# sahaRatul/sela

Hardware: AMD Instinct MI355X
Metric: Msamples/s encode+decode, 16-bit stereo 44.1kHz, 1/2/4/8 GPU; bit-exact vs CPU (higher is better)
Workload: dtype f64+int64

## Files before the change

### sela_amd/csrc/sela_synth.h

```cpp
#ifndef SELA_SYNTH_H_
#define SELA_SYNTH_H_

#include "sela_device.h"

namespace sela {

typedef const volatile __attribute__((address_space(3))) uint64_t* LdsTable;

__device__ __forceinline__ int32_t rice_value(uint32_t ones, uint32_t field, uint32_t k)
{
    const uint32_t rem = k ? (__brev(field) >> (32 - k)) : 0u;
    const uint32_t u = (ones << k) | rem;
    return (int32_t)((u >> 1) ^ (0u - (u & 1u)));
}

struct StreamWords {
    const uint32_t* words;
    uint32_t n_words;
};
__device__ __forceinline__ __amdgpu_buffer_rsrc_t stream_rsrc(const StreamWords& s)
{
    return __builtin_amdgcn_make_buffer_rsrc(
        reinterpret_cast<void*>(read_first_lane(reinterpret_cast<uint64_t>(s.words))), 0,
        4u * (uint32_t)__builtin_amdgcn_readfirstlane((int)s.n_words), 0x00020000);
}
__device__ __forceinline__ void window64(__amdgpu_buffer_rsrc_t rs, uint32_t p, uint32_t& x0, uint32_t& x1)
{
    const uint32_t b = 4 * (p >> 5), sh = p & 31;
    const uint32_t w0 = __builtin_amdgcn_raw_buffer_load_b32(rs, b, 0, 0), w1 = __builtin_amdgcn_raw_buffer_load_b32(rs, b + 4, 0, 0),
                   w2 = __builtin_amdgcn_raw_buffer_load_b32(rs, b + 8, 0, 0);
    x0 = __builtin_amdgcn_alignbit(w1, w0, sh);
    x1 = __builtin_amdgcn_alignbit(w2, w1, sh);
}

template <bool kFold, bool kShift>
__device__ __forceinline__ void synth_mac(uint32_t& zl, uint32_t& zh, uint64_t coef, int32_t s_i, int32_t& shifted)
{
    const int32_t al = (int32_t)(uint32_t)coef, ah = (int32_t)(uint32_t)(coef >> 32);
    const uint64_t z = ((uint64_t)zh << 32) | zl;
    const uint64_t lo = (uint64_t)((int64_t)z + (int64_t)al * (int64_t)s_i);
    if (kFold) {
        if (kShift)
            asm("v_mad_i32_i24 %0, %2, %3, %4\n\tv_ashrrev_i32 %1, 3, %0" : "=v"(zh), "=v"(shifted) : "v"(ah), "s"(s_i), "v"((uint32_t)(lo >> 32)));
        else
            asm("v_mad_i32_i24 %0, %1, %2, %3" : "=v"(zh) : "v"(ah), "s"(s_i), "v"((uint32_t)(lo >> 32)));
    } else {
        zh = (uint32_t)(lo >> 32) + (uint32_t)ah * (uint32_t)s_i;
        if (kShift) {
            shifted = (int32_t)zh >> 3;
            asm volatile("" : "+v"(shifted));
        }
    }
    zl = (uint32_t)lo;
}

constexpr int kAhead = 4;

template <int R, bool kFold, int G, bool kVecShift, int M>
__device__ __forceinline__ void synth_steps(uint32_t& cl, uint32_t& ch, uint32_t& ol, uint32_t& oh, uint32_t& kept,
    LdsTable tab_lane, int32_t r_block, uint32_t four, uint32_t zero, uint64_t (&pf_c)[kAhead], uint64_t (&pf_o)[kAhead], int32_t& shifted)
{
    const int32_t pred = kVecShift ? __builtin_amdgcn_readlane(shifted, M) : __builtin_amdgcn_readlane((int)ch, M) >> 3;
    int32_t m_i;
    if (kFold)
        m_i = pred;
    else
        m_i = (int32_t)((uint32_t)pred - (uint32_t)__builtin_amdgcn_readlane(r_block, M));
    synth_mac<kFold, kVecShift>(cl, ch, pf_c[M % kAhead], m_i, shifted);
    if (R == 2) {
        int32_t unused;
        synth_mac<kFold, false>(ol, oh, pf_o[M % kAhead], m_i, unused);
    }
    if constexpr (M + kAhead < 64) {
        pf_c[M % kAhead] = tab_lane[64 * R - (M + kAhead)];
        if (R == 2)
            pf_o[M % kAhead] = tab_lane[64 - (M + kAhead)];
    }
    if constexpr ((M + 1) % G == 0) {
        constexpr int first_lane = M + 1 - G;
        constexpr int row_mask = 1 << (first_lane / 16);
        constexpr int bank_mask = G == 16 ? 0xf : 1 << ((first_lane % 16) / 4);
        kept = (uint32_t)__builtin_amdgcn_update_dpp((int)kept, (int)ch, 0xE4 , row_mask, bank_mask, false);
        ch = (uint32_t)__builtin_amdgcn_update_dpp((int)ch, (int)four, 0xE4, row_mask, bank_mask, false);
        cl = (uint32_t)__builtin_amdgcn_update_dpp((int)cl, (int)zero, 0xE4, row_mask, bank_mask, false);
    }
    __builtin_amdgcn_sched_barrier(0);
    if constexpr (M < 63)
        synth_steps<R, kFold, G, kVecShift, M + 1>(cl, ch, ol, oh, kept, tab_lane, r_block, four, zero, pf_c, pf_o, shifted);
}

template <int R, bool kFold, int G, bool kVecShift>
__device__ __forceinline__ bool synth_block(int32_t r_block, int32_t& s, uint32_t& cl, uint32_t& ch, uint32_t& ol, uint32_t& oh,
    LdsTable tab_lane, uint32_t four, uint32_t zero)
{
    uint64_t pf_c[kAhead], pf_o[kAhead];
#pragma unroll
    for (int m = 0; m < kAhead; m++) {
        pf_c[m] = tab_lane[64 * R - m];
        pf_o[m] = R == 2 ? tab_lane[64 - m] : 0;
    }
    if (kFold)
        ch -= (uint32_t)r_block << 3;
    uint32_t kept = 0;
    int32_t shifted = 0;
    if (kVecShift) {
        shifted = (int32_t)ch >> 3;
        asm volatile("" : "+v"(shifted));
    }
    __builtin_amdgcn_sched_barrier(0);
    synth_steps<R, kFold, G, kVecShift, 0>(cl, ch, ol, oh, kept, tab_lane, r_block, four, zero, pf_c, pf_o, shifted);
    s = (int32_t)((kFold ? 0u : (uint32_t)r_block) - (uint32_t)((int32_t)kept >> 3));
    return !kFold || !__any((uint32_t)(s + (1 << 23) - 1) >= (1u << 24) - 1u);
}

template <bool kOut32>
struct SynthOut {
};
template <>
struct SynthOut<true> {
    int32_t* samples;
    uint32_t n;
};

template <int R, int G, bool kVecShift, bool kOut32 = false>
__device__ __attribute__((noinline)) void synthesize(
    const uint32_t* words, uint32_t n_words, uint32_t k, uint16_t* pos_smp, const int32_t* ws,
    const uint64_t* tab, bool fold, int lane, SynthOut<kOut32> out32 = SynthOut<kOut32>())
{
    static_assert(G == 4 || G == 16, "groups are DPP banks or rows");
    const StreamWords sw = { words, n_words };
    const __amdgpu_buffer_rsrc_t rs = stream_rsrc(sw);
    k = (uint32_t)__builtin_amdgcn_readfirstlane((int)k);
    const uint32_t kmask = k ? (0xFFFFFFFFu >> (32 - k)) : 0u;
    const bool jit = read_first_lane(reinterpret_cast<uint64_t>(ws)) == 0;
    uint32_t zl[2], zh[2];
#pragma unroll
    for (int h = 0; h < 2; h++) {
        zl[h] = 0;
        zh[h] = 4;
    }
    uint32_t four = 4, zero = 0;
    asm volatile("" : "+v"(four), "+v"(zero));
    const LdsTable tab_lane = (LdsTable)(tab + lane);
    uint32_t p = 0, w0 = 0, w1 = 0, w2 = 0;
    int32_t r_ws = 0;
    uint32_t n_samples = (uint32_t)kBlock;
    if constexpr (kOut32)
        n_samples = (uint32_t)__builtin_amdgcn_readfirstlane((int)out32.n);
    const int n_blocks = kOut32 ? (int)((n_samples + 63) / 64) : kBlock / 64;
    auto issue = [&](int blk) {
        if (jit) {
            p = pos_smp[64 * blk + lane];
            const uint32_t b = 4 * (p >> 5);
            w0 = __builtin_amdgcn_raw_buffer_load_b32(rs, b, 0, 0);
            w1 = __builtin_amdgcn_raw_buffer_load_b32(rs, b + 4, 0, 0);
            w2 = __builtin_amdgcn_raw_buffer_load_b32(rs, b + 8, 0, 0);
        } else if constexpr (kOut32) {
            r_ws = (uint32_t)(64 * blk + lane) < n_samples ? ws[64 * blk + lane] : 0;
        } else {
            w2 = (uint32_t)ws[64 * blk + lane];
        }
    };
    auto land = [&]() -> int32_t {
        if (!jit)
            return kOut32 ? r_ws : (int32_t)w2;
        uint32_t x0 = __builtin_amdgcn_alignbit(w1, w0, p & 31), x1 = __builtin_amdgcn_alignbit(w2, w1, p & 31), ones = 0;
        while (__any(x0 == 0xFFFFFFFFu)) {
            const bool more = x0 == 0xFFFFFFFFu;
            ones += more ? 32u : 0u;
            p += more ? 32u : 0u;
            window64(rs, p, x0, x1);
        }
        const uint32_t t = (uint32_t)__builtin_ctz(~x0);
        const uint32_t field = (uint32_t)(((((uint64_t)x1) << 32) | x0) >> (t + 1)) & kmask;
        return rice_value(ones + t, field, k);
    };
    auto run_block = [&](int blk, uint32_t& cl, uint32_t& ch, uint32_t& ol, uint32_t& oh) {
        const int32_t r_block = land();
        if (blk + 1 < n_blocks)
            issue(blk + 1);
        int32_t s;
        bool done = false;
        fold = fold && !__any((uint32_t)(r_block + (1 << 23) - 1) >= (1u << 24) - 1u);
        if (fold) {
            const uint32_t s0 = cl, s1 = ch, s2 = ol, s3 = oh;
            done = synth_block<R, true, G, kVecShift>(r_block, s, cl, ch, ol, oh, tab_lane, four, zero);
            if (!done) {
                cl = s0, ch = s1;
                if (R == 2)
                    ol = s2, oh = s3;
                fold = false;
            }
        }
        if (!done)
            synth_block<R, false, G, kVecShift>(r_block, s, cl, ch, ol, oh, tab_lane, four, zero);
        if constexpr (kOut32) {
            if ((uint32_t)(64 * blk + lane) < n_samples)
                out32.samples[64 * blk + lane] = s;
        } else
            reinterpret_cast<int16_t*>(pos_smp)[64 * blk + lane] = (int16_t)(uint16_t)(uint32_t)s;
    };
    if (n_blocks > 0)
        issue(0);
    if constexpr (kOut32) {
#pragma unroll 1
        for (int pair = 0; pair < n_blocks; pair += R) {
            run_block(pair, zl[0], zh[0], zl[R - 1], zh[R - 1]);
            if (R == 2 && pair + 1 < n_blocks)
                run_block(pair + 1, zl[1], zh[1], zl[0], zh[0]);
        }
    } else {
#pragma unroll 1
        for (int blk = 0; blk < n_blocks; blk++) {
            run_block(blk, zl[0], zh[0], zl[R - 1], zh[R - 1]);
            if (R == 2) {
                const uint32_t tl = zl[0], th = zh[0];
                zl[0] = zl[1], zh[0] = zh[1];
                zl[1] = tl, zh[1] = th;
            }
        }
    }
    wave_sync();
}

template <bool kVecShift, bool kOut32 = false>
__device__ __forceinline__ void synthesize_by_order(uint32_t order, const uint32_t* words, uint32_t n_words, uint32_t k, uint16_t* pos_smp,
    const int32_t* ws, const uint64_t* tab, bool fold, int lane, SynthOut<kOut32> out32 = SynthOut<kOut32>())
{
    if (order <= 48)
        synthesize<1, 16, kVecShift, kOut32>(words, n_words, k, pos_smp, ws, tab, fold, lane, out32);
    else if (order <= 60)
        synthesize<1, 4, kVecShift, kOut32>(words, n_words, k, pos_smp, ws, tab, fold, lane, out32);
    else
        synthesize<2, 16, kVecShift, kOut32>(words, n_words, k, pos_smp, ws, tab, fold, lane, out32);
}

__device__ inline bool build_synth_table(const int64_t* a, uint64_t* tab, int order, int lane)
{
    uint64_t c[2];
    bool fits = true;
#pragma unroll
    for (int h = 0; h < 2; h++) {
        const int d = lane + 64 * h;
        const uint64_t nv = (uint64_t)(d >= 1 && d <= order ? a[d] : 0);
        const int32_t al = (int32_t)(uint32_t)nv;
        const int32_t ah = (int32_t)(uint32_t)((nv - (uint64_t)(int64_t)al) >> 32);
        fits &= ah >= -(1 << 23) && ah < (1 << 23);
        c[h] = ((uint64_t)(uint32_t)ah << 32) | (uint32_t)al;
    }
    wave_sync();
    if (order <= 60) {
        tab[lane] = c[0];
        tab[lane + 64] = c[0];
    } else {
        tab[lane] = c[0];
        tab[lane + 64] = c[1];
        tab[lane + 128] = c[0];
    }
    wave_sync();
    return !__any(!fits);
}

}

#endif
```

Baseline: 18080.

## Recycle synth lanes via exec-masked moves, add 8-lane groups, streamline rice decode

In the non-out32 path, lane recycling now sets exec with s_bfm_b64 and uses a 64-bit v_mov to restore the accumulator pair, replacing three DPP updates. A G=8 group size is added for orders 49-56, so the lane-recycling granularity can match the order more closely. The rice decode in the jit path also drops the mask and branch on k. The trade-offs are reliance on inline asm that writes exec directly, and a k==0 shift edge case in the new rice code.

```diff
diff --git a/sela_amd/csrc/sela_synth.h b/sela_amd/csrc/sela_synth.h
--- a/sela_amd/csrc/sela_synth.h
+++ b/sela_amd/csrc/sela_synth.h
@@ -54,11 +54,16 @@
     zl = (uint32_t)lo;
 }
 
+struct Restart {
+    uint32_t four, zero;
+    uint64_t sum;
+};
+
 constexpr int kAhead = 4;
 
-template <int R, bool kFold, int G, bool kVecShift, int M>
+template <int R, bool kFold, int G, bool kVecShift, bool kDppRecycle, int M>
 __device__ __forceinline__ void synth_steps(uint32_t& cl, uint32_t& ch, uint32_t& ol, uint32_t& oh, uint32_t& kept,
-    LdsTable tab_lane, int32_t r_block, uint32_t four, uint32_t zero, uint64_t (&pf_c)[kAhead], uint64_t (&pf_o)[kAhead], int32_t& shifted)
+    LdsTable tab_lane, int32_t r_block, const Restart& restart, uint64_t (&pf_c)[kAhead], uint64_t (&pf_o)[kAhead], int32_t& shifted)
 {
     const int32_t pred = kVecShift ? __builtin_amdgcn_readlane(shifted, M) : __builtin_amdgcn_readlane((int)ch, M) >> 3;
     int32_t m_i;
@@ -78,20 +83,29 @@
     }
     if constexpr ((M + 1) % G == 0) {
         constexpr int first_lane = M + 1 - G;
-        constexpr int row_mask = 1 << (first_lane / 16);
-        constexpr int bank_mask = G == 16 ? 0xf : 1 << ((first_lane % 16) / 4);
-        kept = (uint32_t)__builtin_amdgcn_update_dpp((int)kept, (int)ch, 0xE4 , row_mask, bank_mask, false);
-        ch = (uint32_t)__builtin_amdgcn_update_dpp((int)ch, (int)four, 0xE4, row_mask, bank_mask, false);
-        cl = (uint32_t)__builtin_amdgcn_update_dpp((int)cl, (int)zero, 0xE4, row_mask, bank_mask, false);
+        if constexpr (kDppRecycle) {
+            constexpr int row_mask = 1 << (first_lane / 16);
+            constexpr int bank_mask = G == 16 ? 0xf : G == 8 ? 0x3 << ((first_lane % 16) / 8 * 2) : 1 << ((first_lane % 16) / 4);
+            kept = (uint32_t)__builtin_amdgcn_update_dpp((int)kept, (int)ch, 0xE4 , row_mask, bank_mask, false);
+            ch = (uint32_t)__builtin_amdgcn_update_dpp((int)ch, (int)restart.four, 0xE4, row_mask, bank_mask, false);
+            cl = (uint32_t)__builtin_amdgcn_update_dpp((int)cl, (int)restart.zero, 0xE4, row_mask, bank_mask, false);
+        } else {
+            uint64_t c = ((uint64_t)ch << 32) | cl;
+            asm volatile("s_bfm_b64 exec, %4, %5\n\tv_mov_b32 %1, %2\n\tv_mov_b64 %0, %3\n\ts_mov_b64 exec, -1"
+                         : "+v"(c), "+v"(kept)
+                         : "v"(ch), "s"(restart.sum), "n"(G), "n"(first_lane));
+            cl = (uint32_t)c;
+            ch = (uint32_t)(c >> 32);
+        }
     }
     __builtin_amdgcn_sched_barrier(0);
     if constexpr (M < 63)
-        synth_steps<R, kFold, G, kVecShift, M + 1>(cl, ch, ol, oh, kept, tab_lane, r_block, four, zero, pf_c, pf_o, shifted);
-}
-
-template <int R, bool kFold, int G, bool kVecShift>
+        synth_steps<R, kFold, G, kVecShift, kDppRecycle, M + 1>(cl, ch, ol, oh, kept, tab_lane, r_block, restart, pf_c, pf_o, shifted);
+}
+
+template <int R, bool kFold, int G, bool kVecShift, bool kDppRecycle>
 __device__ __forceinline__ bool synth_block(int32_t r_block, int32_t& s, uint32_t& cl, uint32_t& ch, uint32_t& ol, uint32_t& oh,
-    LdsTable tab_lane, uint32_t four, uint32_t zero)
+    LdsTable tab_lane, const Restart& restart)
 {
     uint64_t pf_c[kAhead], pf_o[kAhead];
 #pragma unroll
@@ -108,7 +122,7 @@
         asm volatile("" : "+v"(shifted));
     }
     __builtin_amdgcn_sched_barrier(0);
-    synth_steps<R, kFold, G, kVecShift, 0>(cl, ch, ol, oh, kept, tab_lane, r_block, four, zero, pf_c, pf_o, shifted);
+    synth_steps<R, kFold, G, kVecShift, kDppRecycle, 0>(cl, ch, ol, oh, kept, tab_lane, r_block, restart, pf_c, pf_o, shifted);
     s = (int32_t)((kFold ? 0u : (uint32_t)r_block) - (uint32_t)((int32_t)kept >> 3));
     return !kFold || !__any((uint32_t)(s + (1 << 23) - 1) >= (1u << 24) - 1u);
 }
@@ -127,7 +141,7 @@
     const uint32_t* words, uint32_t n_words, uint32_t k, uint16_t* pos_smp, const int32_t* ws,
     const uint64_t* tab, bool fold, int lane, SynthOut<kOut32> out32 = SynthOut<kOut32>())
 {
-    static_assert(G == 4 || G == 16, "groups are DPP banks or rows");
+    static_assert(G == 4 || G == 8 || G == 16, "groups are aligned runs of lanes inside a row of 16");
     const StreamWords sw = { words, n_words };
     const __amdgpu_buffer_rsrc_t rs = stream_rsrc(sw);
     k = (uint32_t)__builtin_amdgcn_readfirstlane((int)k);
@@ -139,8 +153,9 @@
         zl[h] = 0;
         zh[h] = 4;
     }
-    uint32_t four = 4, zero = 0;
-    asm volatile("" : "+v"(four), "+v"(zero));
+    Restart restart = { 4, 0, 1ull << 34 };
+    if constexpr (kOut32)
+        asm volatile("" : "+v"(restart.four), "+v"(restart.zero));
     const LdsTable tab_lane = (LdsTable)(tab + lane);
     uint32_t p = 0, w0 = 0, w1 = 0, w2 = 0;
     int32_t r_ws = 0;
@@ -172,6 +187,12 @@
             window64(rs, p, x0, x1);
         }
         const uint32_t t = (uint32_t)__builtin_ctz(~x0);
+        if constexpr (!kOut32) {
+            const uint64_t behind = ((((uint64_t)x1) << 32) | x0) >> (t + 1);
+            const uint32_t rem = __brev((uint32_t)(behind << (32 - k)));
+            const uint32_t u = ((ones + t) << k) | rem;
+            return (int32_t)((u >> 1) ^ (0u - (u & 1u)));
+        }
         const uint32_t field = (uint32_t)(((((uint64_t)x1) << 32) | x0) >> (t + 1)) & kmask;
         return rice_value(ones + t, field, k);
     };
@@ -184,7 +205,7 @@
         fold = fold && !__any((uint32_t)(r_block + (1 << 23) - 1) >= (1u << 24) - 1u);
         if (fold) {
             const uint32_t s0 = cl, s1 = ch, s2 = ol, s3 = oh;
-            done = synth_block<R, true, G, kVecShift>(r_block, s, cl, ch, ol, oh, tab_lane, four, zero);
+            done = synth_block<R, true, G, kVecShift, kOut32>(r_block, s, cl, ch, ol, oh, tab_lane, restart);
             if (!done) {
                 cl = s0, ch = s1;
                 if (R == 2)
@@ -193,7 +214,7 @@
             }
         }
         if (!done)
-            synth_block<R, false, G, kVecShift>(r_block, s, cl, ch, ol, oh, tab_lane, four, zero);
+            synth_block<R, false, G, kVecShift, kOut32>(r_block, s, cl, ch, ol, oh, tab_lane, restart);
         if constexpr (kOut32) {
             if ((uint32_t)(64 * blk + lane) < n_samples)
                 out32.samples[64 * blk + lane] = s;
@@ -229,6 +250,8 @@
 {
     if (order <= 48)
         synthesize<1, 16, kVecShift, kOut32>(words, n_words, k, pos_smp, ws, tab, fold, lane, out32);
+    else if (!kOut32 && order <= 56)
+        synthesize<1, 8, kVecShift, kOut32>(words, n_words, k, pos_smp, ws, tab, fold, lane, out32);
     else if (order <= 60)
         synthesize<1, 4, kVecShift, kOut32>(words, n_words, k, pos_smp, ws, tab, fold, lane, out32);
     else
```

Result: no change. 18090 (median of 2 runs) (+0.0%).
